# ssheybani/baby-vision-curriculum

Measured on AMD Instinct MI355X. Metric: video clips/sec (node) VideoMAE-base 16x224^2 bf16 pretraining, higher is better.
Workload: dtype bf16; 1 GPU; VideoMAE-base (ViT-B/16 encoder, 4-layer decoder), 16x224x224 clips, tubelet 2, 90% tube mask, full training step (fwd + MSE + bwd + GradScaler + SGD-Nesterov); clips_per_gpu=256, global_batch=256, parallelism=dp1, weights=random init N(0,0.02), seed 0

## Files before the change

### baby-vision-curriculum_amd/csrc/attention.hip

```cpp
#include <stdlib.h>

#include "attention.h"

namespace bvc {

#define AS3 __attribute__((address_space(3)))
#define MFMA32(a, b, c) __builtin_amdgcn_mfma_f32_32x32x16_bf16((a), (b), (c), 0, 0, 0)

template <int HD>
__device__ __forceinline__ int swz_dual(int r) {
    if constexpr (HD == 64) return (((r >> 1) & 1) << 2) | ((r >> 2) & 3);
    else return (r >> 2) & 3;
}

template <int HD>
constexpr int pan_w(int p) { return HD - 64 * p >= 64 ? 64 : HD - 64 * p; }
constexpr int img_hd(int hd) { return hd == 80 || hd == 88 ? 96 : hd; }
constexpr uint32_t kDmaZero = 0xfffffff0u;
__device__ __forceinline__ int swz_pw(int pw, int r) { return pw == 64 ? swz_dual<64>(r) : swz_dual<32>(r); }

template <int PW, int NW, int VC = PW / 8>
__device__ __forceinline__ void stage_panel(__amdgpu_buffer_rsrc_t rs, int row0, int ld, int col0, char* lds, int GB, int wave, int lane) {
    constexpr int CPR = PW / 8;
    constexpr int RPP = 64 / CPR;
#pragma unroll
    for (int jj = 0; jj < (PW / 8 + NW - 1) / NW; ++jj) {
        const int j = wave + NW * jj;
        if (NW > PW / 8 && j >= PW / 8) break;
        const int r = RPP * j + lane / CPR;
        const int c = (lane % CPR) ^ swz_dual<PW>(r);
        uint32_t off = (uint32_t)(((size_t)(row0 + r) * ld + col0 + c * 8) * 2);
        if constexpr (VC < CPR) off = c < VC ? off : kDmaZero;
        const uint32_t dst = (uint32_t)((RPP * j >> 4) * GB + ((RPP * j) & 15) * PW * 2);
        glds16(rs, off, __builtin_amdgcn_readfirstlane((uint32_t)(size_t)((AS3 char*)lds) + dst));
    }
}

template <int HD, int NW = 4, int HV = HD>
__device__ __forceinline__ void stage64(__amdgpu_buffer_rsrc_t rs, int row0, int ld, int col0, char* lds,
                                        int wave, int lane) {
    static_assert(HV == HD || (HD == 96 && HV > 64 && HV % 8 == 0), "stage64: a narrower head only on the 96 image");
    if constexpr (HD > 64) {
        stage_panel<64, NW>(rs, row0, ld, col0, lds, 16 * HD * 2, wave, lane);
        stage_panel<pan_w<HD>(1), NW, (HV - 64) / 8>(rs, row0, ld, col0 + 64, lds + 2048, 16 * HD * 2, wave, lane);
        return;
    }
    constexpr int CPR = HD / 8;
    constexpr int RPP = 64 / CPR;
#pragma unroll
    for (int jj = 0; jj < (HD / 8 + NW - 1) / NW; ++jj) {
        const int j = wave + NW * jj;
        if (NW > HD / 8 && j >= HD / 8) break;
        const int r = RPP * j + lane / CPR;
        const int c = (lane % CPR) ^ swz_dual<HD>(r);
        const uint32_t off = (uint32_t)(((size_t)(row0 + r) * ld + col0 + c * 8) * 2);
        glds16(rs, off, __builtin_amdgcn_readfirstlane((uint32_t)(size_t)((AS3 char*)lds) + (uint32_t)j * 1024u));
    }
}

template <int HD>
struct FragAddr {
    uint32_t rows[HD / 16];
    uint32_t tr[HD / 32][2];
};

template <int HD>
__device__ __forceinline__ FragAddr<HD> make_frag_addr(int lane) {
    FragAddr<HD> a;
    if constexpr (HD > 64) {
        constexpr int GB = 16 * HD * 2;
        const int r = lane & 31, h = lane >> 5, rg = r & 15;
#pragma unroll
        for (int st = 0; st < HD / 16; ++st) {
            const int pw = pan_w<HD>(st >> 2);
            a.rows[st] = (r >> 4) * GB + (st >> 2) * 2048 + rg * pw * 2 + (((2 * (st & 3) + h) ^ swz_pw(pw, rg)) << 4);
        }
        const int q = (lane >> 2) & 3, p = lane & 3;
#pragma unroll
        for (int t = 0; t < HD / 32; ++t) {
            const int pw = pan_w<HD>(t >> 1);
            const int col = 32 * (t & 1) + 16 * ((lane >> 4) & 1) + 4 * p;
            const int chunk = col >> 3, within = (col & 7) * 2;
#pragma unroll
            for (int half = 0; half < 2; ++half) {
                const int r0 = 4 * h + q + 8 * half;
// ... 685 lines not shown
                asm volatile("" ::: "memory");
#pragma unroll
                for (int r = 0; r < 16; ++r)
                    if (!key_ok || qb * 32 + acc_row(r, h) >= N) { s[r] = 0.f; dp[r] = 0.f; }
            }
            const bf16x8 p0 = acc_to_frag(s, 0), p1 = acc_to_frag(s, 1);
            const bf16x8 d0 = acc_to_frag(dp, 0), d1 = acc_to_frag(dp, 1);
            {
                AS3 char* blk = (AS3 char*)smem + DST + (kb * 5 + qb) * 2048 + (lane & 31) * 64 + 8 * h;
                const int sw = swz_dual<32>(lane & 31);
                typedef __attribute__((ext_vector_type(2))) unsigned int u32x2;
                union { bf16x8 v; u32x2 u[2]; } w0, w1;
                w0.v = d0; w1.v = d1;
                *reinterpret_cast<AS3 u32x2*>(blk + ((0 ^ sw) << 4)) = w0.u[0];
                *reinterpret_cast<AS3 u32x2*>(blk + ((1 ^ sw) << 4)) = w0.u[1];
                *reinterpret_cast<AS3 u32x2*>(blk + ((2 ^ sw) << 4)) = w1.u[0];
                *reinterpret_cast<AS3 u32x2*>(blk + ((3 ^ sw) << 4)) = w1.u[1];
            }
#pragma unroll
            for (int t = 0; t < HD / 32; ++t) {
                dv[t] = MFMA32(lds_tr<0>(oim, fa.tr[t][0], fa.tr[t][1]), p0, dv[t]);
                dk[t] = MFMA32(lds_tr<0>(qim, fa.tr[t][0], fa.tr[t][1]), d0, dk[t]);
            }
#pragma unroll
            for (int t = 0; t < HD / 32; ++t) {
                dv[t] = MFMA32(lds_tr<KS>(oim, fa.tr[t][0], fa.tr[t][1]), p1, dv[t]);
                dk[t] = MFMA32(lds_tr<KS>(qim, fa.tr[t][0], fa.tr[t][1]), d1, dk[t]);
            }
        }
        if (key_ok) {
            bf16_t* krow = dqkv + (size_t)(b * N + ki) * ld + D + head * HD;
            bf16_t* vrow = krow + D;
#pragma unroll
            for (int t = 0; t < HD / 32; ++t)
#pragma unroll
                for (int g = 0; g < 4; ++g) {
                    const int d = 32 * t + 8 * g + 4 * h;
                    uint2 a = {pack2bf(dk[t][4 * g] * scale, dk[t][4 * g + 1] * scale), pack2bf(dk[t][4 * g + 2] * scale, dk[t][4 * g + 3] * scale)};
                    *reinterpret_cast<uint2*>(krow + d) = a;
                    uint2 e = {pack2bf(dv[t][4 * g], dv[t][4 * g + 1]), pack2bf(dv[t][4 * g + 2], dv[t][4 * g + 3])};
                    *reinterpret_cast<uint2*>(vrow + d) = e;
                }
        }
    }
    __syncthreads();
    if (nxt < nheads) {
        stage_qvo(nxt);
        load_stats(nxt);
    }

    for (int qb = wave; qb < NB; qb += 5) {
        const int qi = qb * 32 + (lane & 31);
        f32x16 dq[HD / 32];
#pragma unroll
        for (int t = 0; t < HD / 32; ++t) dq[t] = zero16();
#pragma unroll
        for (int kb = 0; kb < (NBT > 0 ? NBT : NB); ++kb) {
            const AS3 char* kim = lds + KI + kb * SUB;
            const AS3 char* blk = lds + DST + (kb * 5 + qb) * 2048;
            const bf16x8 b0 = lds_tr<0>(blk, fs.tr[0][0], fs.tr[0][1]);
            const bf16x8 b1 = lds_tr<1024>(blk, fs.tr[0][0], fs.tr[0][1]);
#pragma unroll
            for (int t = 0; t < HD / 32; ++t) dq[t] = MFMA32(lds_tr<0>(kim, fa.tr[t][0], fa.tr[t][1]), b0, dq[t]);
#pragma unroll
            for (int t = 0; t < HD / 32; ++t) dq[t] = MFMA32(lds_tr<KS>(kim, fa.tr[t][0], fa.tr[t][1]), b1, dq[t]);
        }
        if (qi < N) {
            bf16_t* orow = dqkv + (size_t)(b * N + qi) * ld + head * HD;
#pragma unroll
            for (int t = 0; t < HD / 32; ++t)
#pragma unroll
                for (int g = 0; g < 4; ++g) {
                    const int d = 32 * t + 8 * g + 4 * h;
                    uint2 a = {pack2bf(dq[t][4 * g] * scale, dq[t][4 * g + 1] * scale), pack2bf(dq[t][4 * g + 2] * scale, dq[t][4 * g + 3] * scale)};
                    *reinterpret_cast<uint2*>(orow + d) = a;
                }
        }
    }
    __syncthreads();
    if (nxt < nheads) stage_k(nxt);
    }
}

static int xcd_remap() {
#ifdef BVC_EXPERIMENTS
    return getenv("BVC_ATTN_PLAIN_GRID") == nullptr;
#else
    return 1;
#endif
}

static bool head_kernel_enabled() {
#ifdef BVC_EXPERIMENTS
    return getenv("BVC_ATTN_NO_HEAD_KERNEL") == nullptr;
#else
    return true;
#endif
}

template <int HD>
static int fwd_hd(const bf16_t* qkv, bf16_t* ctx, float* lse, int B, int N, int H, hipStream_t stream, float sm_scale) {
    constexpr int HI = img_hd(HD);
    const int D = H * HD;
    const size_t bytes = (size_t)B * N * 3 * D * 2;
    const float scale_log2 = (sm_scale > 0.f ? sm_scale : 1.0f / sqrtf((float)HD)) * 1.4426950408889634f;
#ifdef BVC_EXPERIMENTS
    if (getenv("BVC_ATTN_NW8") != nullptr) {
        const dim3 grid8((unsigned)(((N + 255) / 256) * B * H));
        hipLaunchKernelGGL((attn_fwd_kernel<HD, 8>), grid8, dim3(512), 4 * 64 * HI * 2, stream, qkv, ctx, lse, N, H, D, (uint32_t)bytes, scale_log2,
                           xcd_remap());
        BVC_CHECK_HIP(hipGetLastError());
        return BVC_OK;
    }
#endif
    const dim3 grid((unsigned)(((N + 127) / 128) * B * H));
    hipLaunchKernelGGL((attn_fwd_kernel<HD, 4>), grid, dim3(256), 4 * 64 * HI * 2, stream, qkv, ctx, lse, N, H, D, (uint32_t)bytes, scale_log2,
                       xcd_remap());
    BVC_CHECK_HIP(hipGetLastError());
    return BVC_OK;
}

template <int HD>
static int bwd_hd(const bf16_t* qkv, const bf16_t* ctx, const bf16_t* dctx, const float* lse, float* delta, bf16_t* dqkv, int B,
                  int N, int H, hipStream_t stream, float sm_scale, int parts) {
    constexpr int HI = img_hd(HD);
    const int D = H * HD;
    const size_t bytes = (size_t)B * N * 3 * D * 2;
    const float scale = sm_scale > 0.f ? sm_scale : 1.0f / sqrtf((float)HD), scale_log2 = scale * 1.4426950408889634f;
    const dim3 grid((unsigned)(((N + 127) / 128) * B * H));
    const int remap = xcd_remap();
    if constexpr (HD == 64) {
        if (parts == 3 && N <= 160 && head_kernel_enabled()) {
            constexpr size_t lds = 4 * 192 * HD * 2 + 2 * 192 * 4 + 25 * 2048;
            static bool attr_set = false;
            if (!attr_set) {
                BVC_CHECK_HIP(hipFuncSetAttribute(reinterpret_cast<const void*>(&attn_bwd_head_kernel<HD, 5>),
                                                  hipFuncAttributeMaxDynamicSharedMemorySize, (int)lds));
                BVC_CHECK_HIP(hipFuncSetAttribute(reinterpret_cast<const void*>(&attn_bwd_head_kernel<HD, 0>),
                                                  hipFuncAttributeMaxDynamicSharedMemorySize, (int)lds));
                attr_set = true;
            }
            static int ncu = 0;
            if (ncu == 0) {
                int dev = 0;
                hipDeviceProp_t prop;
                BVC_CHECK_HIP(hipGetDevice(&dev));
                BVC_CHECK_HIP(hipGetDeviceProperties(&prop, dev));
                ncu = prop.multiProcessorCount > 0 ? prop.multiProcessorCount : 256;
            }
            const int nheads = B * H;
            const dim3 g((unsigned)(nheads < ncu ? nheads : ncu));
            if (N > 128)
                hipLaunchKernelGGL((attn_bwd_head_kernel<HD, 5>), g, dim3(320), lds, stream, qkv, dctx, ctx, lse, dqkv, N, H, D, nheads,
                                   (uint32_t)bytes, (uint32_t)((size_t)B * N * D * 2), scale, scale_log2);
            else
                hipLaunchKernelGGL((attn_bwd_head_kernel<HD, 0>), g, dim3(320), lds, stream, qkv, dctx, ctx, lse, dqkv, N, H, D, nheads,
                                   (uint32_t)bytes, (uint32_t)((size_t)B * N * D * 2), scale, scale_log2);
            BVC_CHECK_HIP(hipGetLastError());
            return BVC_OK;
        }
    }
    if (parts & 1) {
#ifdef BVC_EXPERIMENTS
    if (HI == HD && getenv("BVC_ATTN_DQ_W") != nullptr) {
        constexpr int NB = 3;
        const dim3 gridw((unsigned)(((N + 32 * NB - 1) / (32 * NB)) * B * H));
        hipLaunchKernelGGL((attn_bwd_dq_w_kernel<HI, NB>), gridw, dim3(64), kRing * 2 * 32 * HI * 2, stream, qkv, dctx, ctx, lse, delta, dqkv, N, H, D,
                           (uint32_t)bytes, scale, scale_log2, remap);
    } else
#endif
    hipLaunchKernelGGL(attn_bwd_dq_kernel<HD>, grid, dim3(256), 4 * 64 * HI * 2, stream, qkv, dctx, ctx, lse, delta, dqkv, N, H, D,
                       (uint32_t)bytes, scale, scale_log2, remap);
    }
    if (parts & 2) {
    constexpr int lds_dkdv = 2 * (2 * 64 * HI * 2 + 512);
    if constexpr (lds_dkdv > 65536) {
        static bool attr_set = false;
        if (!attr_set) {
            BVC_CHECK_HIP(hipFuncSetAttribute(reinterpret_cast<const void*>(&attn_bwd_dkdv_kernel<HD>),
                                              hipFuncAttributeMaxDynamicSharedMemorySize, lds_dkdv));
            attr_set = true;
        }
    }
    hipLaunchKernelGGL(attn_bwd_dkdv_kernel<HD>, grid, dim3(256), lds_dkdv, stream, qkv, dctx, lse, delta, dqkv, N, H, D,
                       (uint32_t)bytes, (uint32_t)((size_t)B * N * D * 2), (uint32_t)((size_t)B * H * N * 4), scale, scale_log2, remap);
    }
    BVC_CHECK_HIP(hipGetLastError());
    return BVC_OK;
}

static bool attn_hd_ok(int hd) { return hd == 32 || hd == 64 || hd == 80 || hd == 88 || hd == 96 || hd == 128; }

int launch_attn_fwd(const bf16_t* qkv, bf16_t* ctx, float* lse, int B, int N, int H, int head_dim, hipStream_t stream, float sm_scale) {
    BVC_REQUIRE(B > 0 && N > 0 && H > 0, "attn_fwd: empty shape");
    BVC_REQUIRE(attn_hd_ok(head_dim), "attn_fwd: head_dim %d unsupported (32, 64, 80, 88, 96 or 128)", head_dim);
    BVC_REQUIRE((size_t)B * N * 3 * H * head_dim * 2 < 0xffffffffull, "attn_fwd: qkv larger than 4 GiB");
    BVC_REQUIRE(img_hd(head_dim) == head_dim || (size_t)B * N * 3 * H * head_dim * 2 < kDmaZero,
                "attn_fwd: qkv of head_dim %d must stay below 4 GiB - 16 bytes", head_dim);
    switch (head_dim) {
        case 32: return fwd_hd<32>(qkv, ctx, lse, B, N, H, stream, sm_scale);
        case 80: return fwd_hd<80>(qkv, ctx, lse, B, N, H, stream, sm_scale);
        case 88: return fwd_hd<88>(qkv, ctx, lse, B, N, H, stream, sm_scale);
        case 96: return fwd_hd<96>(qkv, ctx, lse, B, N, H, stream, sm_scale);
        case 128: return fwd_hd<128>(qkv, ctx, lse, B, N, H, stream, sm_scale);
        default: return fwd_hd<64>(qkv, ctx, lse, B, N, H, stream, sm_scale);
    }
}

int launch_attn_bwd(const bf16_t* qkv, const bf16_t* ctx, const bf16_t* dctx, const float* lse, float* delta,
                    bf16_t* dqkv, int B, int N, int H, int head_dim, hipStream_t stream, float sm_scale, int parts) {
    BVC_REQUIRE(B > 0 && N > 0 && H > 0, "attn_bwd: empty shape");
    BVC_REQUIRE(attn_hd_ok(head_dim), "attn_bwd: head_dim %d unsupported (32, 64, 80, 88, 96 or 128)", head_dim);
    BVC_REQUIRE((size_t)B * N * 3 * H * head_dim * 2 < 0xffffffffull, "attn_bwd: qkv larger than 4 GiB");
    BVC_REQUIRE(img_hd(head_dim) == head_dim || (size_t)B * N * 3 * H * head_dim * 2 < kDmaZero,
                "attn_bwd: qkv of head_dim %d must stay below 4 GiB - 16 bytes", head_dim);
    switch (head_dim) {
        case 32: return bwd_hd<32>(qkv, ctx, dctx, lse, delta, dqkv, B, N, H, stream, sm_scale, parts);
        case 80: return bwd_hd<80>(qkv, ctx, dctx, lse, delta, dqkv, B, N, H, stream, sm_scale, parts);
        case 88: return bwd_hd<88>(qkv, ctx, dctx, lse, delta, dqkv, B, N, H, stream, sm_scale, parts);
        case 96: return bwd_hd<96>(qkv, ctx, dctx, lse, delta, dqkv, B, N, H, stream, sm_scale, parts);
        case 128: return bwd_hd<128>(qkv, ctx, dctx, lse, delta, dqkv, B, N, H, stream, sm_scale, parts);
        default: return bwd_hd<64>(qkv, ctx, dctx, lse, delta, dqkv, B, N, H, stream, sm_scale, parts);
    }
}

}
```

### baby-vision-curriculum_amd/csrc/gemm.h

```cpp
#pragma once
#include "common.h"
#include "dropgate.h"
#include "../../include/bvc.h"

namespace bvc {

enum GemmLayout { GEMM_NT = BVC_GEMM_NT, GEMM_NN = BVC_GEMM_NN, GEMM_TN = BVC_GEMM_TN };

enum GemmEpilogue {
    EPI_F32 = BVC_EPI_F32,
    EPI_BF16 = BVC_EPI_BF16,
    EPI_GELU = BVC_EPI_GELU,
    EPI_RESID = BVC_EPI_RESID,
    EPI_POS = BVC_EPI_POS,
    EPI_E2D = BVC_EPI_E2D,
    EPI_LOSS = BVC_EPI_LOSS,
    EPI_DGELU = BVC_EPI_DGELU,
    EPI_F32_BF16 = BVC_EPI_F32_BF16,
    EPI_RELU = BVC_EPI_RELU,
    EPI_DRELU = BVC_EPI_DRELU,
    EPI_NCE = BVC_EPI_NCE,
    EPI_NCE_BWD = BVC_EPI_NCE_BWD,
    EPI_RESID_LN = BVC_EPI_RESID_LN,
    EPI_DLN = BVC_EPI_DLN,
    EPI_RESID_GATE = BVC_EPI_RESID_GATE
};

using GemmProblem = bvc_gemm_desc;

constexpr int kMaxGroup = 4;

struct Options { int gemm8 = 0; int dw_overlap = 0; int row_ln = 0; int row_stagger = 1; int deterministic = 0; int head_pad = 0; };
Options& options();

float* det_scratch(size_t floats, hipStream_t stream);
size_t det_scratch_bytes();
int det_scratch_release();

struct DryRun { bool on = false; char name[160] = ""; };
DryRun& dry_run();

int launch_gemm(const GemmProblem* probs, int nprob, GemmLayout layout, int tile_cfg, hipStream_t stream, int stages = -1);

int launch_gemm_gate(const GemmProblem& p, const Gate& gate, int tile_cfg, hipStream_t stream);

int gemm_num_tiles(const GemmProblem& p, int tile_cfg);
int gemm_pick_tile(const GemmProblem* probs, int nprob, int tile_cfg);
bool gemm_row_ln_ok(int M, int N, int K);
constexpr size_t kRowLnPartFloats = 512 * 2 * 384;

}
```

### baby-vision-curriculum_amd/csrc/videomae.hip

```cpp
#include <math.h>
#include <stdarg.h>
#include <stdio.h>
#include <stdlib.h>
#include <string.h>

#include <algorithm>
#include <string>
#include <vector>

#include "stack.h"

namespace bvc {
static thread_local char g_err[1024] = "";
void set_error(const char* fmt, ...) {
    va_list ap;
    va_start(ap, fmt);
    vsnprintf(g_err, sizeof(g_err), fmt, ap);
    va_end(ap);
}
const char* last_error() { return g_err; }
}

using namespace bvc;

// ... 37 lines not shown
    L.e2d_w = L.add("encoder_to_decoder.weight", {Dd, D});
    L.mask_token = L.add("mask_token", {1, 1, Dd});
    for (int i = 0; i < c.decoder_num_hidden_layers; ++i)
        L.dec.push_back(add_layer_params(L, "decoder.decoder_layers." + std::to_string(i) + ".", Dd, c.decoder_intermediate_size, true));
    L.norm_w = L.add("decoder.norm.weight", {Dd});
    L.norm_b = L.add("decoder.norm.bias", {Dd});
    L.head_w = L.add("decoder.head.weight", {P, Dd});
    L.head_b = L.add("decoder.head.bias", {P});
    return L;
}

}

struct bvc_ctx {
    bvc_videomae_config cfg;
    Layout lay;
    int max_batch, nmask, nvis, L, P, Kp;
    Arena arena;
    Work w;
    float *pos_enc, *pos_dec;
    int batch = 0;
    bool have_forward = false;
    bf16_t* wbf;
    bool shadow_valid = false;
    const float* params = nullptr;
    int *vis_idx, *msk_idx, *status;
    bf16_t* Ape;
    Stack enc, dec;
    bf16_t* xe_bf;
    float *meanf, *rstdf;
    bf16_t* lnf;
    float* labels;
    bf16_t* diff;
    float* partial;
    int npartial = 0;
    float *dres_enc, *dres_dec;
    bf16_t* de2d;
};

namespace {

void sinusoid(std::vector<float>& out, int n, int d) {
    out.resize((size_t)n * d);
    for (int p = 0; p < n; ++p)
        for (int j = 0; j < d; ++j) {
            const double ang = (double)p / pow(10000.0, 2.0 * (j / 2) / (double)d);
            out[(size_t)p * d + j] = (float)((j & 1) ? cos(ang) : sin(ang));
        }
}

}

namespace {
int pixel_src(const void* pixels, const bvc_pixel_format* fmt, int channels, PixelSrc* out) {
    PixelSrc px = pixels_f32((const float*)pixels);
    if (fmt && fmt->dtype != BVC_PIXELS_F32) {
        BVC_REQUIRE(fmt->dtype == BVC_PIXELS_U8, "pixel format: dtype %d unknown", fmt->dtype);
        BVC_REQUIRE(channels <= 4, "pixel format: uint8 input supports at most 4 channels");
        px.is_u8 = 1;
        for (int c = 0; c < 4; ++c) {
            BVC_REQUIRE(fmt->std[c] != 0.f || c >= channels, "pixel format: std[%d] is zero", c);
            px.mean[c] = fmt->mean[c];
            px.stdv[c] = c < channels ? fmt->std[c] : 1.f;
        }
    }
    *out = px;
    return BVC_OK;
}
}

extern "C" {

const char* bvc_last_error(void) { return bvc::last_error(); }
const char* bvc_version(void) { return "gfx950;bvc-hip-r5"; }

int bvc_set_option(const char* name, int value) {
    BVC_REQUIRE(name != nullptr, "set_option: null name");
    if (!strcmp(name, "gemm8")) { BVC_REQUIRE(value >= -1 && value <= 1, "set_option: gemm8 takes -1 / 0 / 1"); options().gemm8 = value; }
    else if (!strcmp(name, "dw_overlap")) options().dw_overlap = value != 0;
    else if (!strcmp(name, "row_stagger")) options().row_stagger = value != 0;
    else if (!strcmp(name, "row_ln")) { BVC_REQUIRE(value >= -1 && value <= 1, "set_option: row_ln takes -1 / 0 / 1"); options().row_ln = value; }
    else if (!strcmp(name, "deterministic")) { BVC_REQUIRE(value == 0 || value == 1, "set_option: deterministic takes 0 / 1"); options().deterministic = value; }
    else if (!strcmp(name, "head_pad")) { BVC_REQUIRE(value == 0 || value == 1, "set_option: head_pad takes 0 / 1"); options().head_pad = value; }
    else BVC_REQUIRE(false, "set_option: unknown option '%s'", name);
    return BVC_OK;
}
int bvc_get_option(const char* name) {
    if (name && !strcmp(name, "gemm8")) return options().gemm8;
    if (name && !strcmp(name, "dw_overlap")) return options().dw_overlap;
    if (name && !strcmp(name, "row_ln")) return options().row_ln;
    if (name && !strcmp(name, "row_stagger")) return options().row_stagger;
    if (name && !strcmp(name, "deterministic")) return options().deterministic;
    if (name && !strcmp(name, "head_pad")) return options().head_pad;
    bvc::set_error("get_option: unknown option '%s'", name ? name : "(null)");
    return BVC_ERR_INVALID;
}

int bvc_videomae_param_count(const bvc_videomae_config* cfg) {
    if (!cfg || check_config(*cfg) != BVC_OK) return BVC_ERR_INVALID;
    return (int)make_layout(*cfg).entries.size();
}

int64_t bvc_videomae_param_numel(const bvc_videomae_config* cfg) {
    if (!cfg || check_config(*cfg) != BVC_OK) return BVC_ERR_INVALID;
    return make_layout(*cfg).total;
}

int bvc_videomae_param_info(const bvc_videomae_config* cfg, int index, char* name, int name_cap, int64_t* offset,
                            int64_t* numel, int* ndim, int64_t shape[5]) {
    BVC_REQUIRE(cfg && name && offset && numel && ndim && shape, "param_info: null argument");
    TRY(check_config(*cfg));
    const Layout L = make_layout(*cfg);
    BVC_REQUIRE(index >= 0 && index < (int)L.entries.size(), "param_info: index %d out of range", index);
    const ParamEntry& e = L.entries[index];
    snprintf(name, name_cap, "%s", e.name.c_str());
    *offset = e.offset; *numel = e.numel; *ndim = e.ndim;
    for (int i = 0; i < 5; ++i) shape[i] = e.shape[i];
    return BVC_OK;
}

void bvc_videomae_destroy(bvc_ctx* c) {
    if (!c) return;
    free_work(c->w);
    c->arena.release();
    delete c;
}

int bvc_videomae_create(const bvc_videomae_config* cfg, int max_batch, int num_masked, bvc_ctx** out) {
    BVC_REQUIRE(cfg && out, "create: null argument");
    TRY(check_config(*cfg));
    BVC_REQUIRE(max_batch >= 1, "create: max_batch must be >= 1");
    bvc_ctx* c = new bvc_ctx();
    c->cfg = *cfg;
    c->lay = make_layout(*cfg);
    c->max_batch = max_batch;
    const int g = cfg->image_size / cfg->patch_size;
    c->L = (cfg->num_frames / cfg->tubelet_size) * g * g;
    c->nmask = num_masked;
    c->nvis = c->L - num_masked;
    c->P = cfg->num_channels * cfg->tubelet_size * cfg->patch_size * cfg->patch_size;
    c->Kp = c->P;
    if (!(num_masked >= 1 && c->nvis >= 1)) {
        delete c;
        set_error("create: num_masked=%d must leave at least one visible and one masked token of %d", num_masked, c->L);
        return BVC_ERR_INVALID;
    }
    const size_t B = max_batch, Mv = B * c->nvis, Md = B * c->L, Mm = B * c->nmask;
    const int D = cfg->hidden_size, Dd = cfg->decoder_hidden_size, I = cfg->intermediate_size, Id = cfg->decoder_intermediate_size;
    const int H = cfg->num_attention_heads, Hd = cfg->decoder_num_attention_heads;
    int rc = BVC_OK;
    auto fail = [&](int r) { bvc_videomae_destroy(c); return r; };
    {
        const size_t we = std::max<size_t>(3 * (size_t)H * attn_width(D / H), (size_t)I), wd = std::max<size_t>(3 * (size_t)Hd * attn_width(Dd / Hd), (size_t)Id);
        const size_t ee = Mv * we * 2, ed = Md * wd * 2;
        if (ee >= 0xFFFFFFF0ull || ed >= 0xFFFFFFF0ull) {
            const bool dec = ed >= ee;
            set_error("create: max_batch %d exceeds the 4 GiB operand extent: the %s's %zu tokens x %zu bf16 columns are %.2f GiB; at most %zu clips",
                      max_batch, dec ? "decoder" : "encoder", dec ? Md : Mv, dec ? wd : we, (dec ? ed : ee) / 1073741824.0,
                      (size_t)(0xFFFFFFEFull / std::max((dec ? ed : ee) / B, (size_t)1)));
            delete c;
            return BVC_ERR_INVALID;
        }
    }
#define A(expr) if ((rc = (expr)) != BVC_OK) return fail(rc)
    A(c->arena.alloc(&c->pos_enc, (size_t)c->L * D));
    A(c->arena.alloc(&c->pos_dec, (size_t)c->L * Dd));
    A(c->arena.alloc(&c->wbf, (size_t)c->lay.total));
    A(c->arena.alloc(&c->vis_idx, Mv));
    A(c->arena.alloc(&c->msk_idx, Mm));
    if (hipMemset(c->vis_idx, 0, (size_t)Mv * sizeof(int)) != hipSuccess || hipMemset(c->msk_idx, 0, (size_t)Mm * sizeof(int)) != hipSuccess) {
        set_error("videomae_create: hipMemset of the token lists failed");
        bvc_videomae_destroy(c);
        return BVC_ERR_HIP;
    }
    A(c->arena.alloc(&c->status, 4));
    A(c->arena.alloc(&c->Ape, Mv * c->Kp));
// ... 663 lines not shown
```

### baby-vision-curriculum_amd/probe.py

```python
import ctypes

import torch

from . import _lib, _ops

PEAK_BF16_TFLOPS = 2500.0
PEAK_HBM_GBS = 8000.0


def _time(fn, iters=5, warm=2):
    for _ in range(warm):
        fn()
    e0, e1 = torch.cuda.Event(enable_timing=True), torch.cuda.Event(enable_timing=True)
    e0.record()
    for _ in range(iters):
        fn()
    e1.record()
    torch.cuda.synchronize()
    return e0.elapsed_time(e1) * 1e3 / iters


def _rb(dev, *shape):
    return torch.randn(*shape, device=dev, dtype=torch.bfloat16)

# ... 36 lines not shown
                      ln_dgamma=torch.zeros(N, device=dev), ln_dbeta=torch.zeros(N, device=dev))
            nbytes += (4.0 + 4.0 + 2.0) * M * N
        if epi == "DGELU":
            kw["aux"] = _rb(dev, M, N)
            nbytes += 2.0 * M * N
        if epi in ("POS", "E2D"):
            kw["rowtok"] = (torch.arange(M, device=dev, dtype=torch.int32) % 160) * 9
            kw["pos"] = torch.randn(1568, N, device=dev)
            nbytes += 4.0 * M * N
            if epi == "E2D":
                kw["rin"], kw["rout"] = 160, 1568
        if epi == "LOSS":
            kw["labels"] = torch.randn(M, N, device=dev)
            kw["partial"] = torch.empty(1 << 16, device=dev)
            nbytes += 4.0 * M * N
        d = _ops.gemm_desc(A, Bm, M, N, K, E[epi], C, **kw)
        name = _ops.gemm_kernel_name(d, layout, tile)
        us = _time(lambda: _ops.gemm(d, layout, tile))
        add(name, label, count, us, 2.0 * M * N * K, nbytes)

    def dw_single(label, Mo, No, K, count):
        A, Bm = _rb(dev, K, Mo), _rb(dev, K, No)
        C = torch.zeros(Mo, No, device=dev)
        rs = torch.zeros(Mo, device=dev)
        d = _ops.gemm_desc(A, Bm, Mo, No, K, E["F32"], C, rowsum=rs)
        tile, _ = _ops.plan_dw([d])
        name = _ops.gemm_kernel_name(d, _ops.TN, tile)
        us = _time(lambda: _ops.gemm(d, _ops.TN, tile))
        add(name, label, count, us, 2.0 * Mo * No * K, 2.0 * K * (Mo + No) + 4.0 * Mo * No)

    def dw_group(label, M, Dm, Im, count):
        dy, act, dh, ln2, dqkv = _rb(dev, M, Dm), _rb(dev, M, Im), _rb(dev, M, Im), _rb(dev, M, Dm), _rb(dev, M, 3 * Dm)
        shapes = [(Dm, Im), (Im, Dm), (Dm, Dm), (3 * Dm, Dm)]
        outs = [torch.zeros(s, device=dev) for s in shapes]
        bs = [torch.zeros(s[0], device=dev) for s in shapes]
        ds = [_ops.gemm_desc(dy, act, Dm, Im, M, E["F32"], outs[0], rowsum=bs[0]),
              _ops.gemm_desc(dh, ln2, Im, Dm, M, E["F32"], outs[1], rowsum=bs[1]),
              _ops.gemm_desc(dy, ln2, Dm, Dm, M, E["F32"], outs[2], rowsum=bs[2]),
              _ops.gemm_desc(dqkv, ln2, 3 * Dm, Dm, M, E["F32"], outs[3], rowsum=bs[3])]
        tile, split = _ops.plan_dw(ds)
        name = _ops.gemm_kernel_name(ds, _ops.TN, tile)
        us = _time(lambda: _ops.gemm(ds, _ops.TN, tile), iters=3)
        fl = 2.0 * M * (2 * Dm * Im + 4 * Dm * Dm)
        nb = 2.0 * M * (2 * Dm + 2 * Im + 2 * Dm + Dm + 3 * Dm) + 4.0 * (2 * Dm * Im + 4 * Dm * Dm)
        add(name, f"{label} (tile {tile}, split {split})", count, us, fl, nb)

    NT, NN = _ops.NT, _ops.NN
    fused = bool(_lib.lib().bvc_op_row_ln_selected(Md, Dd, Id, 6))
    one("patch embed", NT, Mv, D, 1536, "POS", 1)
    one("enc qkv", NT, Mv, 3 * D, D, "BF16", 12)
    one("enc proj", NT, Mv, D, D, "RESID", 12)
    one("enc fc1+GELU", NT, Mv, I, D, "GELU", 12)
    one("enc fc2", NT, Mv, D, I, "RESID", 12)
    one("enc->dec", NT, Mv, Dd, D, "E2D", 1)
    one("dec qkv", NT, Md, 3 * Dd, Dd, "BF16", 4)
    if fused:
        one("dec proj + LayerNorm", NT, Md, Dd, Dd, "RESID_LN", 4)
    else:
        one("dec proj", NT, Md, Dd, Dd, "RESID", 4)
    one("dec fc1+GELU", NT, Md, Id, Dd, "GELU", 4)
    if fused:
        one("dec fc2 + next LayerNorm", NT, Md, Dd, Id, "RESID_LN", 3)
        one("dec fc2", NT, Md, Dd, Id, "RESID", 1)
    else:
        one("dec fc2", NT, Md, Dd, Id, "RESID", 4)
    one("head+MSE", NT, Mm, P, Dd, "LOSS", 1)
    one("head dX", NN, Mm, Dd, P, "BF16", 1)
    one("dec dX fc2", NN, Md, Id, Dd, "DGELU", 4)
    one("dec dX fc1 + LayerNorm bwd" if fused else "dec dX fc1", NN, Md, Dd, Id, "DLN" if fused else "BF16", 4)
    one("dec dX proj", NN, Md, Dd, Dd, "BF16", 4)
    one("dec dX qkv + LayerNorm bwd" if fused else "dec dX qkv", NN, Md, Dd, 3 * Dd, "DLN" if fused else "BF16", 4)
    one("enc->dec dX", NN, Mv, D, Dd, "F32_BF16", 1)
    one("enc dX fc2", NN, Mv, I, D, "DGELU", 12)
    one("enc dX fc1", NN, Mv, D, I, "BF16", 12)
    one("enc dX proj", NN, Mv, D, D, "BF16", 12)
    one("enc dX qkv", NN, Mv, D, 3 * D, "BF16", 12)
    dw_single("head dW", P, Dd, Mm, 1)
    dw_single("enc->dec dW", Dd, D, Mv, 1)
    dw_single("patch dW", D, 1536, Mv, 1)
    dw_group("dec layer dW group", Md, Dd, Id, 4)
    dw_group("enc layer dW group", Mv, D, I, 12)


def _attention_rows(dev, B, add):
    lib = _lib.lib()
    st = _lib.current_stream_ptr
    for label, N, H, count in (("enc", 160, 12, 12), ("dec", 1568, 6, 4)):
        Dm = 64 * H
        qkv, ctx, dctx, dqkv = _rb(dev, B * N, 3 * Dm), _rb(dev, B * N, Dm), _rb(dev, B * N, Dm), _rb(dev, B * N, 3 * Dm)
        lse = torch.empty(B * H * N, device=dev)
        delta = torch.empty(B * H * N, device=dev)
        p = lambda t: ctypes.c_void_p(t.data_ptr())
        fwd = lambda: _lib.check(lib.bvc_op_attention_fwd(p(qkv), p(ctx), p(lse), B, N, H, 64, st()), "attention_fwd")
        dq = lambda: _lib.check(lib.bvc_op_attention_bwd_part(p(qkv), p(ctx), p(dctx), p(lse), p(delta), p(dqkv), B, N, H, 64, 1, st()), "attention_bwd dq")
        dkv = lambda: _lib.check(lib.bvc_op_attention_bwd_part(p(qkv), p(ctx), p(dctx), p(lse), p(delta), p(dqkv), B, N, H, 64, 2, st()), "attention_bwd dkdv")
        unit = 2.0 * N * N * 64 * H * B
        tok = 2.0 * B * N * Dm
        add("bvc::attn_fwd_kernel<64>", f"{label} attention fwd", count, _time(fwd), 2 * unit, 4 * tok)
        if N <= 160:
            bwd = lambda: _lib.check(lib.bvc_op_attention_bwd(p(qkv), p(ctx), p(dctx), p(lse), p(delta), p(dqkv), B, N, H, 64, st()), "attention_bwd")
            add(f"bvc::attn_bwd_head_kernel<64, {5 if N > 128 else 0}>", f"{label} attention bwd (whole head: S, dP, dV, dK, dQ)", count, _time(bwd),
                5 * unit, 8 * tok)
            continue
        add("bvc::attn_bwd_dq_kernel<64>", f"{label} attention bwd dQ (S, dP, dQ)", count, _time(dq), 3 * unit, 6 * tok)
        add("bvc::attn_bwd_dkdv_kernel<64>", f"{label} attention bwd dK dV (recomputes S, dP)", count, _time(dkv), 2 * unit, 6 * tok)


def _layernorm_rows(dev, B, add):
    lib = _lib.lib()
    st = _lib.current_stream_ptr
    p = lambda t: ctypes.c_void_p(t.data_ptr())
    fused = bool(lib.bvc_op_row_ln_selected(B * 1568, 384, 1536, 6))
    for label, M, Dm, count, count_bwd in (("enc", B * 160, 768, 24, 24), ("dec", B * 1568, 384, 1 if fused else 8, 0 if fused else 8),
                                           ("final", B * 1408, 384, 1, 1)):
        x, dres = torch.randn(M, Dm, device=dev), torch.randn(M, Dm, device=dev)
        gmm, bta = torch.ones(Dm, device=dev), torch.zeros(Dm, device=dev)
        y, dy, dresb = _rb(dev, M, Dm), _rb(dev, M, Dm), _rb(dev, M, Dm)
        mean, rstd = torch.empty(M, device=dev), torch.empty(M, device=dev)
        dg, db = torch.zeros(Dm, device=dev), torch.zeros(Dm, device=dev)
        ws = torch.empty(int(lib.bvc_op_layernorm_bwd_workspace(M, Dm)), device=dev)
        fwd = lambda: _lib.check(lib.bvc_op_layernorm_fwd(p(x), 0, 0, 0, p(gmm), p(bta), p(y), p(mean), p(rstd), M, Dm, 1e-12, st()), "layernorm_fwd")
        bwd = lambda: _lib.check(lib.bvc_op_layernorm_bwd(p(dy), p(x), 0, 0, 0, p(mean), p(rstd), p(gmm), p(dres), 1, p(dresb), p(dg), p(db),
                                                          p(ws), M, Dm, st()), "layernorm_bwd")
        e = float(M) * Dm
        add("bvc::ln_fwd_kernel", f"{label} LayerNorm fwd", count, _time(fwd), 0.0, 6 * e)
        if count_bwd:
            add("bvc::ln_bwd_kernel (+ ln_param_reduce)", f"{label} LayerNorm bwd", count_bwd, _time(bwd), 0.0, 16 * e)


def step_kernels(batch, device):
    rows = {}

    def add(kernel, label, count, us, flops, nbytes):
        r = rows.setdefault(kernel, {"kernel": kernel, "launches_per_step": 0, "us_per_step": 0.0, "flops": 0.0, "bytes": 0.0, "products": []})
        r["launches_per_step"] += count
        r["us_per_step"] += count * us
        r["flops"] += count * flops
        r["bytes"] += count * nbytes
        r["products"].append({"name": label, "launches": count, "launch_us": round(us, 1),
                              "tflops": round(flops / us / 1e6, 1), "gb_per_s": round(nbytes / us / 1e3, 1)})

    with torch.no_grad():
        _gemm_rows(device, batch, add)
        _attention_rows(device, batch, add)
        _layernorm_rows(device, batch, add)
    torch.cuda.empty_cache()
    out = sorted(rows.values(), key=lambda r: -r["us_per_step"])
    total = sum(r["us_per_step"] for r in out)
    for r in out:
        us = r["us_per_step"]
        t_mfma, t_hbm = r["flops"] / (PEAK_BF16_TFLOPS * 1e6), r["bytes"] / (PEAK_HBM_GBS * 1e3)
        r["share_of_probed"] = round(us / total, 4)
        r["tflops"] = round(r["flops"] / us / 1e6, 1)
        r["gb_per_s"] = round(r["bytes"] / us / 1e3, 1)
        r["bound"] = "hbm" if t_hbm > t_mfma else "mfma"
        r["frac"] = round(max(t_mfma, t_hbm) / us, 4)
        r["us_per_step"] = round(us, 1)
        r["algorithmic_flops"] = r.pop("flops")
        r["algorithmic_bytes"] = r.pop("bytes")
    return out, total
```

Before: 3242 clips/s.

## Add 10-wave whole-head attention backward kernel with double-buffered K staging

Adds a new whole-head attention backward kernel for the encoder (N≤160, head_dim 64) that runs 640 threads (10 waves) per block instead of 320. Each pair of waves splits one 32-row key/query block by half of the head dimension, so the dK/dV and dQ work per block is spread over twice as many waves. K is double-buffered in LDS so the next head's K can be staged while the current head is computed. It becomes the default through a new attn_head_waves option. In exchange it uses more LDS and one block per CU, and each wave does less MFMA work, which could increase overhead.

```diff
diff --git a/baby-vision-curriculum_amd/csrc/attention.hip b/baby-vision-curriculum_amd/csrc/attention.hip
--- a/baby-vision-curriculum_amd/csrc/attention.hip
+++ b/baby-vision-curriculum_amd/csrc/attention.hip
@@ -1,6 +1,7 @@
 #include <stdlib.h>
 
 #include "attention.h"
+#include "gemm.h"
 
 namespace bvc {
 
@@ -852,6 +853,203 @@
     }
 }
 
+template <int HD, int NBT>
+__global__ __launch_bounds__(640, 1) void attn_bwd_head10_kernel(const bf16_t* __restrict__ qkv, const bf16_t* __restrict__ dctx,
+                                                                 const bf16_t* __restrict__ ctx, const float* __restrict__ lse,
+                                                                 bf16_t* __restrict__ dqkv, int N, int H, int D, int nheads,
+                                                                 uint32_t qkv_bytes, uint32_t dctx_bytes, float scale, float scale_log2) {
+    static_assert(HD == 64, "whole-head backward: head_dim 64");
+    extern __shared__ __attribute__((aligned(16))) char smem[];
+    constexpr int IR = NBT > 0 ? 32 * NBT : 128;
+    constexpr int IMG = IR * HD * 2, SUB = 32 * HD * 2, KS = 16 * HD * 2;
+    constexpr int QI = 0, KI = IMG, VI = 3 * IMG, OI = 4 * IMG;
+    constexpr int STAT = 5 * IMG;
+    constexpr int DST = STAT + 2 * 192 * 4;
+    const AS3 char* lds = (const AS3 char*)smem;
+    const int tid = threadIdx.x, lane = tid & 63;
+    const int wave = __builtin_amdgcn_readfirstlane(tid >> 6);
+    const int pair = wave >> 1, th = wave & 1;
+    const int ld = 3 * D, h = lane >> 5;
+    const int NB = NBT > 0 ? NBT : (N + 31) >> 5;
+    const __amdgpu_buffer_rsrc_t rq = make_rsrc(qkv, qkv_bytes), rd = make_rsrc(dctx, dctx_bytes);
+    const FragAddr<HD> fa = make_frag_addr<HD>(lane);
+    const FragAddr<32> fs = make_frag_addr<32>(lane);
+    const uint32_t tr0 = th ? fa.tr[1][0] : fa.tr[0][0], tr1 = th ? fa.tr[1][1] : fa.tr[0][1];
+
+    auto stage_img = [&](__amdgpu_buffer_rsrc_t rs, int row0, int ldr, int col0, int img) __attribute__((always_inline)) {
+#pragma unroll
+        for (int jj = 0; jj < (IR / 8 + 9) / 10; ++jj) {
+            const int j = wave + 10 * jj;
+            if (j >= 4 * NB) break;
+            const int r = 8 * j + (lane >> 3);
+            const int c = (lane & 7) ^ swz_dual<HD>(r);
+            const uint32_t off = (uint32_t)(((size_t)(row0 + r) * ldr + col0 + c * 8) * 2);
+            glds16(rs, off, __builtin_amdgcn_readfirstlane((uint32_t)(size_t)((AS3 char*)smem) + (uint32_t)(img + j * 1024)));
+        }
+    };
+    auto stage_qvo = [&](int bh) __attribute__((always_inline)) {
+        const int b = bh / H, head = bh % H, row0 = b * N;
+        stage_img(rq, row0, ld, head * HD, QI);
+        stage_img(rq, row0, ld, 2 * D + head * HD, VI);
+        stage_img(rd, row0, D, head * HD, OI);
+    };
+    auto stage_k = [&](int bh, int buf) __attribute__((always_inline)) {
+        const int b = bh / H, head = bh % H, row0 = b * N;
+        stage_img(rq, row0, ld, D + head * HD, KI + buf * IMG);
+    };
+    float st_lse = 0.f, st_del[2];
+    auto load_stats = [&](int bh) __attribute__((always_inline)) {
+        const int b = bh / H, head = bh % H;
+        st_lse = (tid < N) ? lse[(size_t)bh * N + tid] : 0.f;
+#pragma unroll
+        for (int k = 0; k < 2; ++k) {
+            const int q = (tid >> 3) + 80 * k, c = tid & 7;
+            float acc = 0.f;
+            if (q < N) {
+                const bf16x8 dv = load8(dctx + (size_t)(b * N + q) * D + head * HD + 8 * c);
+                const bf16x8 ov = load8(ctx + (size_t)(b * N + q) * D + head * HD + 8 * c);
+#pragma unroll
+                for (int j = 0; j < 8; ++j) acc += bf2f((bf16_t)dv[j]) * bf2f((bf16_t)ov[j]);
+            }
+            st_del[k] = acc;
+        }
+    };
+    auto store_stats = [&]() __attribute__((always_inline)) {
+        AS3 float* st = (AS3 float*)((AS3 char*)smem + STAT);
+        if (tid < 192) st[tid] = st_lse;
+#pragma unroll
+        for (int k = 0; k < 2; ++k) {
+            float acc = st_del[k];
+            acc += __shfl_xor(acc, 1, 64);
+            acc += __shfl_xor(acc, 2, 64);
+            acc += __shfl_xor(acc, 4, 64);
+            const int q = (tid >> 3) + 80 * k;
+            if ((tid & 7) == 0) st[192 + q] = -acc;
+        }
+    };
+
+    int bh = blockIdx.x;
+    if (bh >= nheads) return;
+    load_stats(bh);
+    stage_qvo(bh);
+    stage_k(bh, 0);
+    int kbuf = 0;
+    for (; bh < nheads; bh += gridDim.x, kbuf ^= 1) {
+    const int b = bh / H, head = bh % H;
+    const int nxt = bh + gridDim.x;
+    const int KB = KI + kbuf * IMG;
+    asm volatile("s_waitcnt vmcnt(0)" ::: "memory");
+    store_stats();
+    __syncthreads();
+    if (nxt < nheads) stage_k(nxt, kbuf ^ 1);
+
+    if (pair < NB) {
+        const int kb = pair;
+        const int ki = kb * 32 + (lane & 31);
+        bf16x8 kf[HD / 16], vf[HD / 16];
+#pragma unroll
+        for (int st = 0; st < HD / 16; ++st) {
+            kf[st] = *reinterpret_cast<const AS3 bf16x8*>(lds + KB + kb * SUB + fa.rows[st]);
+            vf[st] = *reinterpret_cast<const AS3 bf16x8*>(lds + VI + kb * SUB + fa.rows[st]);
+        }
+        f32x16 dk = zero16(), dv = zero16();
+        const bool key_ok = ki < N;
+#pragma unroll
+        for (int qb = 0; qb < (NBT > 0 ? NBT : NB); ++qb) {
+            const AS3 char* qim = lds + QI + qb * SUB;
+            const AS3 char* oim = lds + OI + qb * SUB;
+            const AS3 float* stl = reinterpret_cast<const AS3 float*>(lds + STAT) + qb * 32 + 4 * h;
+            f32x16 s = zero16(), dp;
+#pragma unroll
+            for (int g = 0; g < 4; ++g) {
+                const f32x4 nd = *reinterpret_cast<const AS3 f32x4*>(stl + 192 + 8 * g);
+#pragma unroll
+                for (int e = 0; e < 4; ++e) dp[4 * g + e] = nd[e];
+            }
+#pragma unroll
+            for (int stp = 0; stp < HD / 16; ++stp) {
+                s = MFMA32(*reinterpret_cast<const AS3 bf16x8*>(qim + fa.rows[stp]), kf[stp], s);
+                dp = MFMA32(*reinterpret_cast<const AS3 bf16x8*>(oim + fa.rows[stp]), vf[stp], dp);
+            }
+#pragma unroll
+            for (int g = 0; g < 4; ++g) {
+                const f32x4 ls = *reinterpret_cast<const AS3 f32x4*>(stl + 8 * g);
+#pragma unroll
+                for (int e = 0; e < 4; ++e) {
+                    const int r = 4 * g + e;
+                    const float pr = fast_exp2(fmaf(s[r], scale_log2, -ls[e]));
+                    s[r] = pr;
+                    dp[r] = pr * dp[r];
+                }
+            }
+            const bool qrag = NBT > 0 ? qb == NBT - 1 : true;
+            if ((qrag && qb * 32 + 32 > N) || !__all(key_ok)) {
+                asm volatile("" ::: "memory");
+#pragma unroll
+                for (int r = 0; r < 16; ++r)
+                    if (!key_ok || (qrag && qb * 32 + acc_row(r, h) >= N)) { s[r] = 0.f; dp[r] = 0.f; }
+            }
+            const bf16x8 p0 = acc_to_frag(s, 0), p1 = acc_to_frag(s, 1);
+            const bf16x8 d0 = acc_to_frag(dp, 0), d1 = acc_to_frag(dp, 1);
+            {
+                AS3 char* blk = (AS3 char*)smem + DST + (kb * 5 + qb) * 2048 + (lane & 31) * 64 + 8 * h;
+                const int sw = swz_dual<32>(lane & 31);
+                typedef __attribute__((ext_vector_type(2))) unsigned int u32x2;
+                union { bf16x8 v; u32x2 u[2]; } w;
+                w.v = th ? d1 : d0;
+                *reinterpret_cast<AS3 u32x2*>(blk + (((2 * th) ^ sw) << 4)) = w.u[0];
+                *reinterpret_cast<AS3 u32x2*>(blk + (((2 * th + 1) ^ sw) << 4)) = w.u[1];
+            }
+            dv = MFMA32(lds_tr<0>(oim, tr0, tr1), p0, dv);
+            dk = MFMA32(lds_tr<0>(qim, tr0, tr1), d0, dk);
+            dv = MFMA32(lds_tr<KS>(oim, tr0, tr1), p1, dv);
+            dk = MFMA32(lds_tr<KS>(qim, tr0, tr1), d1, dk);
+        }
+        if (key_ok) {
+            bf16_t* krow = dqkv + (size_t)(b * N + ki) * ld + D + head * HD + 32 * th;
+            bf16_t* vrow = krow + D;
+#pragma unroll
+            for (int g = 0; g < 4; ++g) {
+                const int d = 8 * g + 4 * h;
+                uint2 a = {pack2bf(dk[4 * g] * scale, dk[4 * g + 1] * scale), pack2bf(dk[4 * g + 2] * scale, dk[4 * g + 3] * scale)};
+                *reinterpret_cast<uint2*>(krow + d) = a;
+                uint2 e = {pack2bf(dv[4 * g], dv[4 * g + 1]), pack2bf(dv[4 * g + 2], dv[4 * g + 3])};
+                *reinterpret_cast<uint2*>(vrow + d) = e;
+            }
+        }
+    }
+    __syncthreads();
+    if (nxt < nheads) {
+        stage_qvo(nxt);
+        load_stats(nxt);
+    }
+
+    if (pair < NB) {
+        const int qb = pair;
+        const int qi = qb * 32 + (lane & 31);
+        f32x16 dq = zero16();
+#pragma unroll
+        for (int kb = 0; kb < (NBT > 0 ? NBT : NB); ++kb) {
+            const AS3 char* kim = lds + KB + kb * SUB;
+            const AS3 char* blk = lds + DST + (kb * 5 + qb) * 2048;
+            const bf16x8 b0 = lds_tr<0>(blk, fs.tr[0][0], fs.tr[0][1]);
+            const bf16x8 b1 = lds_tr<1024>(blk, fs.tr[0][0], fs.tr[0][1]);
+            dq = MFMA32(lds_tr<0>(kim, tr0, tr1), b0, dq);
+            dq = MFMA32(lds_tr<KS>(kim, tr0, tr1), b1, dq);
+        }
+        if (qi < N) {
+            bf16_t* orow = dqkv + (size_t)(b * N + qi) * ld + head * HD + 32 * th;
+#pragma unroll
+            for (int g = 0; g < 4; ++g) {
+                const int d = 8 * g + 4 * h;
+                uint2 a = {pack2bf(dq[4 * g] * scale, dq[4 * g + 1] * scale), pack2bf(dq[4 * g + 2] * scale, dq[4 * g + 3] * scale)};
+                *reinterpret_cast<uint2*>(orow + d) = a;
+            }
+        }
+    }
+    }
+}
+
 static int xcd_remap() {
 #ifdef BVC_EXPERIMENTS
     return getenv("BVC_ATTN_PLAIN_GRID") == nullptr;
@@ -901,6 +1099,35 @@
     const int remap = xcd_remap();
     if constexpr (HD == 64) {
         if (parts == 3 && N <= 160 && head_kernel_enabled()) {
+            static int ncu = 0;
+            if (ncu == 0) {
+                int dev = 0;
+                hipDeviceProp_t prop;
+                BVC_CHECK_HIP(hipGetDevice(&dev));
+                BVC_CHECK_HIP(hipGetDeviceProperties(&prop, dev));
+                ncu = prop.multiProcessorCount > 0 ? prop.multiProcessorCount : 256;
+            }
+            const int nheads = B * H;
+            const dim3 g((unsigned)(nheads < ncu ? nheads : ncu));
+            if (options().attn_head_waves == 10) {
+                constexpr size_t lds5 = 5 * 160 * HD * 2 + 2 * 192 * 4 + 25 * 2048, lds0 = 5 * 128 * HD * 2 + 2 * 192 * 4 + 25 * 2048;
+                static bool attr10_set = false;
+                if (!attr10_set) {
+                    BVC_CHECK_HIP(hipFuncSetAttribute(reinterpret_cast<const void*>(&attn_bwd_head10_kernel<HD, 5>),
+                                                      hipFuncAttributeMaxDynamicSharedMemorySize, (int)lds5));
+                    BVC_CHECK_HIP(hipFuncSetAttribute(reinterpret_cast<const void*>(&attn_bwd_head10_kernel<HD, 0>),
+                                                      hipFuncAttributeMaxDynamicSharedMemorySize, (int)lds0));
+                    attr10_set = true;
+                }
+                if (N > 128)
+                    hipLaunchKernelGGL((attn_bwd_head10_kernel<HD, 5>), g, dim3(640), lds5, stream, qkv, dctx, ctx, lse, dqkv, N, H, D, nheads,
+                                       (uint32_t)bytes, (uint32_t)((size_t)B * N * D * 2), scale, scale_log2);
+                else
+                    hipLaunchKernelGGL((attn_bwd_head10_kernel<HD, 0>), g, dim3(640), lds0, stream, qkv, dctx, ctx, lse, dqkv, N, H, D, nheads,
+                                       (uint32_t)bytes, (uint32_t)((size_t)B * N * D * 2), scale, scale_log2);
+                BVC_CHECK_HIP(hipGetLastError());
+                return BVC_OK;
+            }
             constexpr size_t lds = 4 * 192 * HD * 2 + 2 * 192 * 4 + 25 * 2048;
             static bool attr_set = false;
             if (!attr_set) {
@@ -910,16 +1137,6 @@
                                                   hipFuncAttributeMaxDynamicSharedMemorySize, (int)lds));
                 attr_set = true;
             }
-            static int ncu = 0;
-            if (ncu == 0) {
-                int dev = 0;
-                hipDeviceProp_t prop;
-                BVC_CHECK_HIP(hipGetDevice(&dev));
-                BVC_CHECK_HIP(hipGetDeviceProperties(&prop, dev));
-                ncu = prop.multiProcessorCount > 0 ? prop.multiProcessorCount : 256;
-            }
-            const int nheads = B * H;
-            const dim3 g((unsigned)(nheads < ncu ? nheads : ncu));
             if (N > 128)
                 hipLaunchKernelGGL((attn_bwd_head_kernel<HD, 5>), g, dim3(320), lds, stream, qkv, dctx, ctx, lse, dqkv, N, H, D, nheads,
                                    (uint32_t)bytes, (uint32_t)((size_t)B * N * D * 2), scale, scale_log2);
diff --git a/baby-vision-curriculum_amd/csrc/gemm.h b/baby-vision-curriculum_amd/csrc/gemm.h
--- a/baby-vision-curriculum_amd/csrc/gemm.h
+++ b/baby-vision-curriculum_amd/csrc/gemm.h
@@ -30,7 +30,7 @@
 
 constexpr int kMaxGroup = 4;
 
-struct Options { int gemm8 = 0; int dw_overlap = 0; int row_ln = 0; int row_stagger = 1; int deterministic = 0; int head_pad = 0; };
+struct Options { int gemm8 = 0; int dw_overlap = 0; int row_ln = 0; int row_stagger = 1; int deterministic = 0; int head_pad = 0; int attn_head_waves = 10; };
 Options& options();
 
 float* det_scratch(size_t floats, hipStream_t stream);
diff --git a/baby-vision-curriculum_amd/csrc/videomae.hip b/baby-vision-curriculum_amd/csrc/videomae.hip
--- a/baby-vision-curriculum_amd/csrc/videomae.hip
+++ b/baby-vision-curriculum_amd/csrc/videomae.hip
@@ -143,6 +143,7 @@
     else if (!strcmp(name, "row_ln")) { BVC_REQUIRE(value >= -1 && value <= 1, "set_option: row_ln takes -1 / 0 / 1"); options().row_ln = value; }
     else if (!strcmp(name, "deterministic")) { BVC_REQUIRE(value == 0 || value == 1, "set_option: deterministic takes 0 / 1"); options().deterministic = value; }
     else if (!strcmp(name, "head_pad")) { BVC_REQUIRE(value == 0 || value == 1, "set_option: head_pad takes 0 / 1"); options().head_pad = value; }
+    else if (!strcmp(name, "attn_head_waves")) { BVC_REQUIRE(value == 5 || value == 10, "set_option: attn_head_waves takes 5 / 10"); options().attn_head_waves = value; }
     else BVC_REQUIRE(false, "set_option: unknown option '%s'", name);
     return BVC_OK;
 }
@@ -153,6 +154,7 @@
     if (name && !strcmp(name, "row_stagger")) return options().row_stagger;
     if (name && !strcmp(name, "deterministic")) return options().deterministic;
     if (name && !strcmp(name, "head_pad")) return options().head_pad;
+    if (name && !strcmp(name, "attn_head_waves")) return options().attn_head_waves;
     bvc::set_error("get_option: unknown option '%s'", name ? name : "(null)");
     return BVC_ERR_INVALID;
 }
diff --git a/baby-vision-curriculum_amd/probe.py b/baby-vision-curriculum_amd/probe.py
--- a/baby-vision-curriculum_amd/probe.py
+++ b/baby-vision-curriculum_amd/probe.py
@@ -142,6 +142,11 @@
     dw_group("enc layer dW group", Mv, D, I, 12)
 
 
+def head_bwd_kernel_name(N, waves):
+    nbt = 5 if N > 128 else 0
+    return f"bvc::attn_bwd_head10_kernel<64, {nbt}>" if waves == 10 else f"bvc::attn_bwd_head_kernel<64, {nbt}>"
+
+
 def _attention_rows(dev, B, add):
     lib = _lib.lib()
     st = _lib.current_stream_ptr
@@ -159,7 +164,7 @@
         add("bvc::attn_fwd_kernel<64>", f"{label} attention fwd", count, _time(fwd), 2 * unit, 4 * tok)
         if N <= 160:
             bwd = lambda: _lib.check(lib.bvc_op_attention_bwd(p(qkv), p(ctx), p(dctx), p(lse), p(delta), p(dqkv), B, N, H, 64, st()), "attention_bwd")
-            add(f"bvc::attn_bwd_head_kernel<64, {5 if N > 128 else 0}>", f"{label} attention bwd (whole head: S, dP, dV, dK, dQ)", count, _time(bwd),
+            add(head_bwd_kernel_name(N, lib.bvc_get_option(b"attn_head_waves")), f"{label} attention bwd (whole head: S, dP, dV, dK, dQ)", count, _time(bwd),
                 5 * unit, 8 * tok)
             continue
         add("bvc::attn_bwd_dq_kernel<64>", f"{label} attention bwd dQ (S, dP, dQ)", count, _time(dq), 3 * unit, 6 * tok)
```

New measurement: 3258 clips/s, median of 6. No clear change (+0.5%).
